# AIM-Harvard/pyradiomics

Measured on AMD Instinct MI355X. Metric: Mvoxels/s for GLCM+GLRLM build, 512^3 vol @32 bins, higher is better.
Workload: dtype u8 levels / u32 counts / f64 out; 1 GPU; GLCM+GLRLM matrix build, 512^3 int32+uint8 volume resident in HBM, 32 grey levels, full mask, 13 angles, uniform levels; one volume per GPU (batch sharding, no collective); size=512, levels=32, dist=uniform, deferred_mode=pipeline

## Files before the change

### pyradiomics_amd/csrc/kernels_sweep.h

```cpp
#pragma once
#include "prad_runtime.h"

namespace prad {

typedef unsigned int u32;
typedef unsigned long long u64;

__global__ void __launch_bounds__(256) pack_levels_kernel(const int *__restrict__ image,
                                                          const uint8_t *__restrict__ mask, long long n, int NX,
                                                          int pitch, int padw, int Ng,
                                                          uint8_t *__restrict__ levels, int *__restrict__ flags,
                                                          int vec_ok, int shift, uint8_t *__restrict__ rowzero = nullptr) {
  const long long tid = (long long)blockIdx.x * blockDim.x + threadIdx.x;
  const long long nthreads = (long long)gridDim.x * blockDim.x;
  const bool linear = (padw == 0 && pitch == NX);
  int bad = 0;
  long long done = 0;
  if (vec_ok) {
    const long long n16 = n >> 4;
    const int upr = NX >> 4;
    const int4 *im4 = reinterpret_cast<const int4 *>(image);
    const uint4 *mk4 = reinterpret_cast<const uint4 *>(mask);
    for (long long t = tid; t < n16; t += nthreads) {
      const uint4 m = mk4[t];
// ... 462 lines not shown
  Walker<DO_GLCM, DO_GLRLM, LONG, FUSED> w[LPL];
#pragma unroll
  for (int j = 0; j < LPL; j++) w[j].init(lds, h, Nr, glrlm_acc + (size_t)D.slot * Ng * Nr, lane);
  bool seen_multi = false;
  const int lane4 = lane * LPL;
  const int NM = D.NM, NU = D.NU, NX = D.NX, du = D.du, dx = D.dx;
  const long long sU = D.sU;
  WrapGeo geo;
  geo.du = du; geo.dx = dx; geo.NU = NU; geo.NX = NX;
  geo.delta = D.sM + (long long)du * D.sU + dx;
  geo.uwrapfix = -(long long)du * NU * D.sU;

  (void)nwaves;
  for (;;) {
    int grabbed = 0;
    if (lane == 0) grabbed = atomicAdd(&work[blockIdx.y], 1);
    const int chunk = __builtin_amdgcn_readfirstlane(grabbed);
    if (chunk >= D.chunks) break;
    const int u0 = chunk / D.LXc;
    const int xfirst = (chunk - u0 * D.LXc) * CW;
    bool dead[LPL];
    bool anydead_l = false;
#pragma unroll
    for (int j = 0; j < LPL; j++) {
      dead[j] = xfirst + lane4 + j >= NX;
      anydead_l = anydead_l || dead[j];
    }
    const bool anydead = __ballot(anydead_l) != 0;
    u32 livemask = 0;
#pragma unroll
    for (int j = 0; j < LPL; j++) livemask |= dead[j] ? 0u : (0xffu << (8 * j));
#pragma unroll
    for (int j = 0; j < LPL; j++) w[j].begin_line();

    WrapPos pos;
    pos.off = (long long)u0 * sU + xfirst;
    pos.u = u0;
    pos.b = xfirst;
    pos.ent_sb = -1;
    pos.ent_uw = false;
    int t0 = 0;
    for (; t0 + U <= NM; t0 += U) {
      u32 v[U];
      bool risky_l = false;
#pragma unroll
      for (int j = 0; j < LPL; j++) risky_l = risky_l || w[j].risky(U);
      const bool quiet = !pos.ent_uw && pos.ent_sb < 0 && wrap_quiet<CW>(pos, geo, U);
      if (quiet) {
        const uint8_t *pl = L + pos.off + lane4;
#pragma unroll
        for (int k = 0; k < U; k++) {
          v[k] = load_lines<LPL>(pl);
          pl += geo.delta;
        }
        if (anydead) {
#pragma unroll
          for (int k = 0; k < U; k++) v[k] &= livemask;
        }
        pos.off += (long long)U * geo.delta;
        pos.u += U * du;
        pos.b += U * dx;
        if (LONG && __ballot(risky_l) != 0) {
#pragma unroll
          for (int k = 0; k < U; k++) {
#pragma unroll
            for (int j = 0; j < LPL; j++) w[j].template step<true>((int)((v[k] >> (8 * j)) & 0xffu));
          }
        } else {
          steps_plain_group<LPL, U>(w, v);
        }
      } else {
        int sb[U];
        bool uw[U];
#pragma unroll
        for (int k = 0; k < U; k++) {
          v[k] = load_lines<LPL>(L + pos.off + lane4) & livemask;
          sb[k] = pos.ent_sb;
          uw[k] = pos.ent_uw;
          wrap_advance<CW>(pos, geo);
        }
        if (LONG && __ballot(risky_l) != 0) seen_multi |= steps_break_group<LPL, U, true>(w, v, sb, uw, lane4);
        else seen_multi |= steps_break_group<LPL, U, false>(w, v, sb, uw, lane4);
      }
    }
    for (int t = t0; t < NM; t++) {
      const u32 v = load_lines<LPL>(L + pos.off + lane4) & livemask;
#pragma unroll
      for (int j = 0; j < LPL; j++) {
        const bool brk = pos.ent_uw || (pos.ent_sb == lane4 + j);
        const int cur = (int)((v >> (8 * j)) & 0xffu);
        seen_multi |= w[j].step_brk(cur, brk);
      }
      wrap_advance<CW>(pos, geo);
    }
#pragma unroll
    for (int j = 0; j < LPL; j++) seen_multi |= w[j].end_line();
  }
  if (DO_GLRLM && !FUSED && seen_multi) multi[D.slot] = 1;
  flush_block_hist<DO_GLCM, DO_GLRLM, FUSED>(lds, h, Nr, D.slot, glcm_acc, glrlm_acc);
}

#define PRAD_ROW_PITCH 80
template <bool DO_GLCM, bool DO_GLRLM, bool LONG, bool FUSED>
__global__ void __launch_bounds__(512) sweep_rows_kernel(const uint8_t *__restrict__ L, long long nrows, int NX,
                                                         int pitch, int slot, int Ng, int Nr, int RS,
                                                         u32 *__restrict__ glcm_acc, u32 *__restrict__ glrlm_acc,
                                                         int *__restrict__ multi, int *__restrict__ flags) {
  extern __shared__ u32 lds[];
  if (flags[0]) return;
  const HistLayout h = hist_layout(DO_GLCM, DO_GLRLM, FUSED, Ng, RS);
  if (FUSED && (unsigned)(size_t)((lds_u32 *)lds) != 0u) {
    if (threadIdx.x == 0) atomicExch(flags + 2, 1);
    return;
  }
  for (int i = threadIdx.x; i < h.words; i += blockDim.x) lds[i] = 0;
  __syncthreads();
  const int lane = threadIdx.x & 63;
  const int wave = threadIdx.x >> 6;
  const int wpb = blockDim.x >> 6;
  uint8_t *tile = reinterpret_cast<uint8_t *>(lds + ((h.words + 3) & ~3)) + (size_t)wave * 64 * PRAD_ROW_PITCH;
  const long long ngroups = (nrows + 63) / 64;
  const long long nwaves = (long long)gridDim.x * wpb;
  Walker<DO_GLCM, DO_GLRLM, LONG, FUSED> w;
  w.init(lds, h, Nr, glrlm_acc + (size_t)slot * Ng * Nr, lane);
  bool seen_multi = false;
  const bool vec16 = (pitch & 15) == 0 && ((uintptr_t)L & 15) == 0;

  for (long long grp = (long long)blockIdx.x * wpb + wave; grp < ngroups; grp += nwaves) {
    const long long r0 = grp * 64;
    w.begin_line();
    for (int xc = 0; xc < NX; xc += 64) {
      if (vec16) {
#pragma unroll
        for (int j = 0; j < 4; j++) {
          const int rr = j * 16 + (lane >> 2);
          const int cx = xc + (lane & 3) * 16;
          uint4 q = make_uint4(0, 0, 0, 0);
          if (r0 + rr < nrows && cx < NX) {
            q = *reinterpret_cast<const uint4 *>(L + (r0 + rr) * pitch + cx);
            const int valid = NX - cx;
            if (valid < 16) {
              u32 *qw = reinterpret_cast<u32 *>(&q);
#pragma unroll
              for (int wd = 0; wd < 4; wd++) {
                const int keep = valid - 4 * wd;
                qw[wd] = keep >= 4 ? qw[wd] : (keep <= 0 ? 0u : (qw[wd] & ((1u << (8 * keep)) - 1u)));
              }
            }
          }
          *reinterpret_cast<uint4 *>(tile + rr * PRAD_ROW_PITCH + (lane & 3) * 16) = q;
        }
      } else {
        const bool xin = xc + lane < NX;
#pragma unroll 8
        for (int rr = 0; rr < 64; rr++) {
          uint8_t b = 0;
          if (xin && r0 + rr < nrows) b = L[(r0 + rr) * pitch + xc + lane];
          tile[rr * PRAD_ROW_PITCH + lane] = b;
        }
      }
      __builtin_amdgcn_wave_barrier();
      const uint4 *row = reinterpret_cast<const uint4 *>(tile + lane * PRAD_ROW_PITCH);
#pragma unroll
      for (int q = 0; q < 4; q++) {
        const uint4 d = row[q];
        const u32 wds[4] = {d.x, d.y, d.z, d.w};
#pragma unroll
        for (int k = 0; k < 4; k++) {
          if (LONG && __ballot(w.risky(4)) != 0) {
#pragma unroll
            for (int b = 0; b < 4; b++) w.template step<true>((int)((wds[k] >> (8 * b)) & 0xffu));
          } else {
#pragma unroll
            for (int b = 0; b < 4; b++) w.template step<false>((int)((wds[k] >> (8 * b)) & 0xffu));
          }
        }
      }
      __builtin_amdgcn_wave_barrier();
    }
    seen_multi |= w.end_line();
  }
  if (DO_GLRLM && !FUSED && seen_multi) multi[slot] = 1;
  flush_block_hist<DO_GLCM, DO_GLRLM, FUSED>(lds, h, Nr, slot, glcm_acc, glrlm_acc);
}

__global__ void __launch_bounds__(64) glcm_diag_resolve_kernel(const u32 *__restrict__ glcm_acc,
                                                               const u32 *__restrict__ glrlm_acc, int Ng, int Nr,
                                                               int Na, double *__restrict__ glcm_out,
                                                               int *__restrict__ multi) {
  const int i = blockIdx.x, a = blockIdx.y, lane = threadIdx.x;
  const u32 *row = glrlm_acc + ((size_t)a * Ng + i) * Nr;
  unsigned long long pairs = 0;
  int found = 0;
  for (int r = lane; r < Nr; r += 64) {
    const u32 v = row[r];
    pairs += (unsigned long long)r * v;
    found |= (r > 0 && v != 0);
  }
  const u32 *grow = glcm_acc + ((size_t)a * Ng + i) * Ng;
  for (int j = lane; j < Ng; j += 64) found |= (grow[j] != 0);
  for (int o = 32; o > 0; o >>= 1) pairs += __shfl_xor(pairs, o);
  if (lane == 0) glcm_out[((size_t)i * Ng + i) * Na + a] = (double)pairs;
  if (__ballot(found) != 0 && lane == 0) multi[a] = 1;
}

struct AngleSet {
  int count;
  int off[PRAD_MAX_SWEEP][3];
};
template <typename T>
__global__ void __launch_bounds__(256) multi_check_kernel(AngleSet A, const T *__restrict__ L, int Nz, int Ny,
                                                          int Nx, int pitch, int *__restrict__ multi) {
  const int a = blockIdx.y;
  if (multi[a]) return;
  const int dz = A.off[a][0], dy = A.off[a][1], dx = A.off[a][2];
  const long long n = (long long)Nz * Ny * Nx, plane = (long long)Ny * Nx;
  const long long stride = (long long)gridDim.x * blockDim.x;
  for (long long i = (long long)blockIdx.x * blockDim.x + threadIdx.x; i < n; i += stride) {
    int z = (int)(i / plane);
    const int r = (int)(i - (long long)z * plane);
    int y = r / Nx, x = r - y * Nx;
    const int pz = z - dz, py = y - dy, px = x - dx;
    if ((unsigned)pz < (unsigned)Nz && (unsigned)py < (unsigned)Ny && (unsigned)px < (unsigned)Nx) continue;
    int cnt = 0;
    while ((unsigned)z < (unsigned)Nz && (unsigned)y < (unsigned)Ny && (unsigned)x < (unsigned)Nx) {
      cnt += L[((long long)z * Ny + y) * pitch + x] != 0;
      if (cnt > 1) {
        multi[a] = 1;
        return;
      }
      z += dz; y += dy; x += dx;
    }
  }
}

__global__ void finalize_glcm_kernel(const u32 *__restrict__ acc, const u32 *__restrict__ glrlm_acc, int Ng, int Nr,
                                     int Na, int diag_from_runs, double *__restrict__ out) {
  const long long idx = (long long)blockIdx.x * blockDim.x + threadIdx.x;
  const long long total = (long long)Ng * Ng * Na;
  if (idx >= total) return;
  const int a = (int)(idx % Na);
  const long long ij = idx / Na;
  const int i = (int)(ij / Ng), j = (int)(ij - (long long)i * Ng);
  if (diag_from_runs && i == j) return;
  out[idx] = (double)acc[(size_t)a * Ng * Ng + ij];
}

__global__ void __launch_bounds__(256) finalize_glcm_diag_kernel(const u32 *__restrict__ glcm_acc, u32 *glrlm_acc, int Ng, int Nr,
                                                                 int Na, int nb1, double *__restrict__ glcm_out,
                                                                 int *__restrict__ multi, int restore_from = -1) {
  if ((int)blockIdx.x < nb1) {
    const long long idx = (long long)blockIdx.x * blockDim.x + threadIdx.x;
    const long long total = (long long)Ng * Ng * Na;
    if (idx >= total) return;
    const int a = (int)(idx % Na);
    const long long ij = idx / Na;
    const int i = (int)(ij / Ng), j = (int)(ij - (long long)i * Ng);
    if (i == j) return;
    glcm_out[idx] = (double)glcm_acc[(size_t)a * Ng * Ng + ij];
    return;
  }
  const int pair = ((int)blockIdx.x - nb1) * 4 + (int)(threadIdx.x >> 6), lane = threadIdx.x & 63;
  if (pair >= Ng * Na) return;
  const int i = pair % Ng, a = pair / Ng;
  u32 *row = glrlm_acc + ((size_t)a * Ng + i) * Nr;
  unsigned long long pairs = 0, longer = 0;
  int found = 0;
  for (int r = lane; r < Nr; r += 64) {
    const u32 v = row[r];
    pairs += (unsigned long long)r * v;
    if (r > 0) longer += v;
    found |= (r > 0 && v != 0);
  }
  const u32 *grow = glcm_acc + ((size_t)a * Ng + i) * Ng;
  for (int j = lane; j < Ng; j += 64) found |= (grow[j] != 0);
  for (int o = 32; o > 0; o >>= 1) pairs += __shfl_xor(pairs, o);
  if (lane == 0) glcm_out[((size_t)i * Ng + i) * Na + a] = (double)pairs;
  if (__ballot(found) != 0 && lane == 0) multi[a] = 1;
  if (restore_from >= 0 && a != restore_from) {
    const u32 *xrow = glrlm_acc + ((size_t)restore_from * Ng + i) * Nr;
    unsigned long long nvox = 0;
    for (int r = lane; r < Nr; r += 64) nvox += (unsigned long long)(r + 1) * xrow[r];
    for (int o = 32; o > 0; o >>= 1) {
      nvox += __shfl_xor(nvox, o);
      longer += __shfl_xor(longer, o);
    }
    if (lane == 0) row[0] = (u32)(nvox - (pairs + longer));
  }
}

__global__ void finalize_glrlm_kernel(const u32 *__restrict__ acc, const int *__restrict__ multi, int Ng, int Nr,
                                      int Na, double *__restrict__ out, const int *__restrict__ flags = nullptr,
                                      int *__restrict__ sticky = nullptr) {
  if (sticky && blockIdx.x == 0 && threadIdx.x == 0 && (flags[0] || flags[2])) sticky[0] = 1;
  const long long idx = (long long)blockIdx.x * blockDim.x + threadIdx.x;
  const long long total = (long long)Ng * Nr * Na;
  if (idx >= total) return;
  const int a = (int)(idx % Na);
  const long long gr = idx / Na;
  const int r = (int)(gr % Nr);
  out[idx] = (r == 0 && !multi[a]) ? 0.0 : (double)acc[(size_t)a * Ng * Nr + gr];
}

}
```

### pyradiomics_amd/csrc/prad_api.hip

```cpp
#include "prad_runtime.h"
#include "kernels_generic.h"
#include "kernels_pairs.h"
#include "kernels_sweep.h"
#include "kernels_sweepfw.h"
#include "kernels_sweepfw2.h"
#include "kernels_neigh.h"
#include "kernels_glszm.h"
#include "kernels_voxel.h"
#include "kernels_voxslide.h"
#include "kernels_mcc.h"
#include "kernels_voxtex.h"
#include "kernels_binning.h"

#include <algorithm>
#include <atomic>
#include <chrono>
#include <cmath>
#include <condition_variable>
#include <cstdlib>
#include <deque>
#include <limits>
#include <mutex>
#include <thread>

// ... 558 lines not shown
  return launch_lines_lpl<G, R, LNG, F, 1>(k, p, levels, Ng, Nr, glcm_acc, glrlm_acc, multi);
}

template <bool LNG, int K, bool HASPAD, bool PACK>
int launch_fw_kpp(Call &k, const SweepPlan &p, const PackJob &pj, const uint8_t *levels, const uint8_t *rowzero, int Ng, int Nr,
                  u32 *glcm_acc, u32 *glrlm_acc, int *multi, int *flags_d) {
  const size_t lds = p.fw_xblocks > 0 ? std::max(p.lds_fw, p.lds_fw_rows) : p.lds_fw;
  PRAD_HIP(hipFuncSetAttribute(reinterpret_cast<const void *>(&sweep_fw_kernel<LNG, K, HASPAD, PACK>),
                               hipFuncAttributeMaxDynamicSharedMemorySize, (int)lds));
  hipLaunchKernelGGL((sweep_fw_kernel<LNG, K, HASPAD, PACK>), dim3(p.fw_blocks + p.fw_xblocks), dim3(p.fw_threads), lds, k.s, p.fwset, pj,
                     levels, rowzero, Ng, Nr, p.RSfw, glcm_acc, glrlm_acc, multi + 2 * PRAD_MAX_SWEEP + PRAD_FW_WORK_STRIDE, flags_d);
  return check_launch("sweep_fw_kernel");
}
template <bool LNG, int K, bool HASPAD>
int launch_fw_kp(Call &k, const SweepPlan &p, const PackJob &pj, const uint8_t *levels, const uint8_t *rowzero, int Ng, int Nr,
                 u32 *glcm_acc, u32 *glrlm_acc, int *multi, int *flags_d) {
  if (pj.n16 > 0) return launch_fw_kpp<LNG, K, HASPAD, true>(k, p, pj, levels, rowzero, Ng, Nr, glcm_acc, glrlm_acc, multi, flags_d);
  return launch_fw_kpp<LNG, K, HASPAD, false>(k, p, pj, levels, rowzero, Ng, Nr, glcm_acc, glrlm_acc, multi, flags_d);
}
template <bool LNG, int K>
int launch_fw_k(Call &k, const SweepPlan &p, const PackJob &pj, const uint8_t *levels, const uint8_t *rowzero, int Ng, int Nr,
                u32 *glcm_acc, u32 *glrlm_acc, int *multi, int *flags_d) {
  if (p.Nx != 64 * K) return launch_fw_kp<LNG, K, true>(k, p, pj, levels, rowzero, Ng, Nr, glcm_acc, glrlm_acc, multi, flags_d);
  return launch_fw_kp<LNG, K, false>(k, p, pj, levels, rowzero, Ng, Nr, glcm_acc, glrlm_acc, multi, flags_d);
}
int launch_fw(Call &k, const SweepPlan &p, const PackJob &pj, const uint8_t *levels, const uint8_t *rowzero, int Ng, int Nr,
              u32 *glcm_acc, u32 *glrlm_acc, int *multi, int *flags_d) {
  if (p.fwK == 16)
    return p.LONGfw ? launch_fw_k<true, 16>(k, p, pj, levels, rowzero, Ng, Nr, glcm_acc, glrlm_acc, multi, flags_d)
                    : launch_fw_k<false, 16>(k, p, pj, levels, rowzero, Ng, Nr, glcm_acc, glrlm_acc, multi, flags_d);
  if (p.LONGfw) return p.fwK == 4 ? launch_fw_k<true, 4>(k, p, pj, levels, rowzero, Ng, Nr, glcm_acc, glrlm_acc, multi, flags_d)
                                : launch_fw_k<true, 8>(k, p, pj, levels, rowzero, Ng, Nr, glcm_acc, glrlm_acc, multi, flags_d);
  return p.fwK == 4 ? launch_fw_k<false, 4>(k, p, pj, levels, rowzero, Ng, Nr, glcm_acc, glrlm_acc, multi, flags_d)
                    : launch_fw_k<false, 8>(k, p, pj, levels, rowzero, Ng, Nr, glcm_acc, glrlm_acc, multi, flags_d);
}

template <bool LNG, int K, bool HASPAD, bool SKIP1, bool PACK>
int launch_fw2_khsp(Call &k, const SweepPlan &p, const PackJob &pj, const uint8_t *levels16, int Ng, int Nr, u32 *glcm_acc, u32 *glrlm_acc,
                    int *work, int *flags_d) {
  PRAD_HIP(hipFuncSetAttribute(reinterpret_cast<const void *>(&sweep_fw2_kernel<LNG, K, HASPAD, SKIP1, PACK>),
                               hipFuncAttributeMaxDynamicSharedMemorySize, (int)p.lds_fw2));
  hipLaunchKernelGGL((sweep_fw2_kernel<LNG, K, HASPAD, SKIP1, PACK>), dim3(p.fw_blocks), dim3(1024), p.lds_fw2, k.s, p.fwset, pj, levels16,
                     Ng, Nr, p.RS2, p.fw2_copies, glcm_acc, glrlm_acc, work, flags_d);
  return check_launch("sweep_fw2_kernel");
}
template <bool LNG, int K, bool HASPAD, bool SKIP1>
int launch_fw2_khs(Call &k, const SweepPlan &p, const PackJob &pj, const uint8_t *levels16, int Ng, int Nr, u32 *glcm_acc, u32 *glrlm_acc,
                   int *work, int *flags_d) {
  if (pj.n16 > 0) return launch_fw2_khsp<LNG, K, HASPAD, SKIP1, true>(k, p, pj, levels16, Ng, Nr, glcm_acc, glrlm_acc, work, flags_d);
  return launch_fw2_khsp<LNG, K, HASPAD, SKIP1, false>(k, p, pj, levels16, Ng, Nr, glcm_acc, glrlm_acc, work, flags_d);
}
template <bool LNG, int K>
int launch_fw2_k(Call &k, const SweepPlan &p, const PackJob &pj, const uint8_t *levels16, int Ng, int Nr, u32 *glcm_acc, u32 *glrlm_acc,
                 int *multi, int *flags_d) {
  int *work = multi + 2 * PRAD_MAX_SWEEP + PRAD_FW_WORK_STRIDE;
  if (p.Nx != 64 * K)
    return p.skip1 ? launch_fw2_khs<LNG, K, true, true>(k, p, pj, levels16, Ng, Nr, glcm_acc, glrlm_acc, work, flags_d)
                   : launch_fw2_khs<LNG, K, true, false>(k, p, pj, levels16, Ng, Nr, glcm_acc, glrlm_acc, work, flags_d);
  return p.skip1 ? launch_fw2_khs<LNG, K, false, true>(k, p, pj, levels16, Ng, Nr, glcm_acc, glrlm_acc, work, flags_d)
                 : launch_fw2_khs<LNG, K, false, false>(k, p, pj, levels16, Ng, Nr, glcm_acc, glrlm_acc, work, flags_d);
}
int launch_fw2(Call &k, const SweepPlan &p, const PackJob &pj, const uint8_t *levels16, int Ng, int Nr, u32 *glcm_acc, u32 *glrlm_acc,
               int *multi, int *flags_d) {
  if (p.LONGfw2) return p.fwK == 4 ? launch_fw2_k<true, 4>(k, p, pj, levels16, Ng, Nr, glcm_acc, glrlm_acc, multi, flags_d)
                                 : launch_fw2_k<true, 8>(k, p, pj, levels16, Ng, Nr, glcm_acc, glrlm_acc, multi, flags_d);
  return p.fwK == 4 ? launch_fw2_k<false, 4>(k, p, pj, levels16, Ng, Nr, glcm_acc, glrlm_acc, multi, flags_d)
                    : launch_fw2_k<false, 8>(k, p, pj, levels16, Ng, Nr, glcm_acc, glrlm_acc, multi, flags_d);
}

template <bool LNG>
int launch_fw_rows(Call &k, const SweepPlan &p, const uint8_t *levels, int Ng, int Nr, u32 *glcm_acc, u32 *glrlm_acc, int *flags_d) {
  const long long nrows = (long long)p.Nz * p.Ny, groups = fw_row_groups(nrows);
  const int wpb = p.fw_rows_threads / 64;
  const unsigned gx = (unsigned)std::max<long long>(1, std::min<long long>((groups + wpb - 1) / wpb, (long long)cu_count()));
  PRAD_HIP(hipFuncSetAttribute(reinterpret_cast<const void *>(&sweep_fw_rows_kernel<LNG>),
                               hipFuncAttributeMaxDynamicSharedMemorySize, (int)p.lds_fw_rows));
  hipLaunchKernelGGL((sweep_fw_rows_kernel<LNG>), dim3(gx), dim3(p.fw_rows_threads), p.lds_fw_rows, k.s, levels, nrows, p.Nx,
                     p.pitch, p.row_slot, Ng, Nr, p.RSfw_rows, glcm_acc, glrlm_acc, flags_d);
  return check_launch("sweep_fw_rows_kernel");
}

template <bool LNG>
int launch_fw2_rows(Call &k, const SweepPlan &p, const uint8_t *levels16, int Ng, int Nr, u32 *glcm_acc, u32 *glrlm_acc, int *flags_d) {
  const long long nrows = (long long)p.Nz * p.Ny, groups = nrows >= 4096 ? ((nrows + 511) / 512) * 8 : (nrows + 63) / 64;
  const int wpb = p.fw2r_waves;
  const unsigned gx = (unsigned)std::max<long long>(1, std::min<long long>((groups + wpb - 1) / wpb, (long long)cu_count()));
  PRAD_HIP(hipFuncSetAttribute(reinterpret_cast<const void *>(&sweep_fw2_rows_kernel<LNG>),
                               hipFuncAttributeMaxDynamicSharedMemorySize, (int)p.lds_fw2_rows));
  hipLaunchKernelGGL((sweep_fw2_rows_kernel<LNG>), dim3(gx), dim3(64 * wpb), p.lds_fw2_rows, k.s, levels16, nrows, p.Nx, p.pitch16,
                     p.row_slot, Ng, Nr, p.RS2r, p.fw2r_copies, glcm_acc, glrlm_acc, flags_d);
  return check_launch("sweep_fw2_rows_kernel");
}

template <bool G, bool R, bool LNG, bool F>
int launch_rows(Call &k, const SweepPlan &p, const uint8_t *levels, int Ng, int Nr, u32 *glcm_acc, u32 *glrlm_acc,
                int *multi) {
  const long long nrows = (long long)p.Nz * p.Ny;
  const long long groups = (nrows + 63) / 64;
  const int wpb = kRowsThreads / 64;
  const int per_cu = std::max(1, std::min(2048 / kRowsThreads, (int)(160 * 1024 / p.lds_bytes_rows)));
  const unsigned gx = (unsigned)std::max<long long>(1, std::min<long long>((groups + wpb - 1) / wpb, (long long)cu_count() * per_cu));
  PRAD_HIP(hipFuncSetAttribute(reinterpret_cast<const void *>(&sweep_rows_kernel<G, R, LNG, F>),
                               hipFuncAttributeMaxDynamicSharedMemorySize, (int)p.lds_bytes_rows));
  hipLaunchKernelGGL((sweep_rows_kernel<G, R, LNG, F>), dim3(gx), dim3(kRowsThreads), p.lds_bytes_rows, k.s, levels,
                     nrows, p.Nx, p.pitch, p.row_slot, Ng, Nr, p.RSr, glcm_acc, glrlm_acc, multi, k.flags_d);
  return check_launch("sweep_rows_kernel");
}

__global__ void __launch_bounds__(256) zero3_kernel(u32 *__restrict__ a, size_t na, u32 *__restrict__ b, size_t nb,
                                                    u32 *__restrict__ c3, size_t nc) {
  const size_t t = (size_t)blockIdx.x * blockDim.x + threadIdx.x, nt = (size_t)gridDim.x * blockDim.x;
  uint4 *a4 = reinterpret_cast<uint4 *>(a);
  for (size_t i = t; i < na / 4; i += nt) a4[i] = make_uint4(0, 0, 0, 0);
  for (size_t i = (na & ~(size_t)3) + t; i < na; i += nt) a[i] = 0;
  for (size_t i = t; i < nb; i += nt) b[i] = 0;
  for (size_t i = t; i < nc; i += nt) c3[i] = 0;
}

struct VolState {
  bool valid = false;
  SweepPlan p;
  int Ng = 0, Nr = 0, Na = 0;
  double *glcm = nullptr, *glrlm = nullptr;
  uint8_t *levels = nullptr, *rowzero = nullptr;
  uint8_t *levels16 = nullptr;
  u32 *acc = nullptr, *glcm_acc = nullptr, *glrlm_acc = nullptr;
  int *multi = nullptr;
  int *flags_d = nullptr;
  bool packed_inline = false;
  int lane = -1;
};

bool fin_side() {
  static const bool on = getenv("PRAD_FINALIZE_STREAM") != nullptr && atoi(getenv("PRAD_FINALIZE_STREAM")) != 0;
  return on;
}
int fin_wait_for_lane(hipStream_t s, int lane);

int vol_prepare(Call &k, const SweepPlan &p, int Ng, int Nr, double *glcm, double *glrlm, VolState &v) {
  Context &c = *k.c;
  if (fin_side() && c.lane >= 0) PRAD_TRY(fin_wait_for_lane(k.s, c.lane));
  v.lane = c.lane;
  v.valid = true;
  v.p = p;
  v.Ng = Ng;
  v.Nr = Nr;
  v.Na = k.Na;
  v.glcm = glcm;
  v.glrlm = glrlm;
  v.flags_d = k.flags_d;
  const long long nrows = (long long)p.Nz * p.Ny;
  v.levels = nullptr;
  if (!(p.fw2 && p.fw2_rows && p.lines.count > 0 && p.row_slot >= 0) || getenv("PRAD_FW2_KEEP8")) {
    PRAD_TRY(c.get<uint8_t>("levels", (size_t)nrows * p.pitch + 1024, &v.levels));
    v.levels += 512;
  }
  v.levels16 = nullptr;
  if (p.fw2) {
    PRAD_TRY(c.get<uint8_t>("levels16", (size_t)nrows * p.pitch16 + 4096, &v.levels16));
    v.levels16 += 2048;
  }
  const size_t nglcm = glcm ? (size_t)k.Na * Ng * Ng : 0, nglrlm = glrlm ? (size_t)k.Na * Ng * Nr : 0;
  const size_t nctl = 2 * PRAD_MAX_SWEEP + (size_t)PRAD_FW_WORK_STRIDE * (PRAD_FW_DOMAINS * PRAD_MAX_SWEEP + 1);
  PRAD_TRY(c.get<u32>("sweep_acc", nglcm + nglrlm + nctl, &v.acc));
  v.glcm_acc = v.acc;
  v.glrlm_acc = v.acc + nglcm;
  v.multi = (int *)(v.acc + nglcm + nglrlm);
  v.rowzero = nullptr;
  if (p.fw) PRAD_TRY(c.get<uint8_t>("rowzero", (size_t)nrows + 64, &v.rowzero));
  const size_t acc_w = nglcm + nglrlm + nctl, rz_w = v.rowzero ? ((size_t)nrows + 3) / 4 : 0;
  const size_t total_w = acc_w + rz_w + 4;
  const unsigned gx = (unsigned)std::max<size_t>(1, std::min<size_t>((total_w / 4 + 255) / 256, 1024));
  hipLaunchKernelGGL(zero3_kernel, dim3(gx), dim3(256), 0, k.s, v.acc, acc_w, reinterpret_cast<u32 *>(v.rowzero), rz_w,
                     reinterpret_cast<u32 *>(v.flags_d), (size_t)4);
  return check_launch("zero3_kernel");
}

bool pipeline_volume(const SweepPlan &p, bool glcm, bool glrlm) {
  if (!(p.ok && p.lines.count > 0 && glcm && glrlm)) return false;
  return (p.fw && p.fused) || (p.fw2 && !getenv("PRAD_FW2_LANES"));
}
bool pack_inline_ok(const Call &k, const VolState &v) {
  if (!(v.glcm && v.glrlm && v.p.pitch == v.p.Nx && v.p.padw == 0 && (k.g.n % 16) == 0 &&
        ((((uintptr_t)k.image) | ((uintptr_t)k.mask) | ((uintptr_t)v.levels)) & 15) == 0))
    return false;
  if (k.g.n >= (1LL << 31)) return false;
  if (v.p.fw2) return v.levels16 && v.p.pitch16 == 2 * v.p.Nx && (((uintptr_t)v.levels16) & 15) == 0;
  return v.p.fw && v.p.fused;
}

PackJob make_pack_job(const Call &k, const VolState &v, const VolState *host) {
  PackJob j;
  memset(&j, 0, sizeof(j));
  j.image = k.image;
  j.mask = k.mask;
  j.levels = v.levels;
  j.levels16 = v.p.fw2 ? v.levels16 : nullptr;
  j.rowzero = v.rowzero;
  j.flags = v.flags_d;
  j.n16 = k.g.n / 16;
  j.NX = v.p.Nx;
  j.Ng = v.Ng;
  double groups = 0, waves = 16.0;
  if (host) {
    for (int i = 0; i < host->p.fwset.count; i++) groups += (double)host->p.fwset.d[i].NM * host->p.fwset.d[i].NU / PRAD_FW_U;
    waves = 16.0 * std::max(1, host->p.fw_blocks);
  }
  const double units = (double)j.n16 / 64.0;
  const double slack = v.p.fw2 ? 1.05 : 0.92;
  j.every = (int)std::max(1.0, std::min(64.0, std::floor(slack * groups / std::max(1.0, units))));
  (void)waves;
  if (const char *e = getenv("PRAD_PACK_EVERY")) j.every = std::max(1, atoi(e));
  return j;
}

int vol_pack_standalone(Call &k, VolState &v) {
  Context &c = *k.c;
  const SweepPlan &p = v.p;
  Timed t(c, "pack", k.s);
  if (p.fw2) {
    const unsigned gx = (unsigned)std::max<long long>(1, std::min<long long>((k.g.n / 4 + 255) / 256, 8192));
    hipLaunchKernelGGL(pack_levels16_kernel, dim3(gx), dim3(256), 0, k.s, k.image, k.mask, k.g.n, p.Nx, p.pitch16, p.pitch, v.Ng,
                       v.levels16, v.levels, v.flags_d);
    return check_launch("pack_levels16_kernel");
  }
  const int vec_ok = p.vec_rows && ((((uintptr_t)k.image) | ((uintptr_t)k.mask) | ((uintptr_t)v.levels)) & 15) == 0;
  const unsigned gx = (unsigned)std::max<long long>(1, std::min<long long>((k.g.n / 16 + 255) / 256, 4096));
  const int shift = (v.glcm && v.glrlm && p.fused) ? PRAD_FUSED_SHIFT : 0;
  hipLaunchKernelGGL(pack_levels_kernel, dim3(gx), dim3(256), 0, k.s, k.image, k.mask, k.g.n, p.Nx, p.pitch, p.padw,
                     v.Ng, v.levels, v.flags_d, vec_ok, shift, v.rowzero);
  return check_launch("pack_levels_kernel");
}

template <bool G, bool R, bool F>
int launch_sweeps(Call &k, const VolState &v, const PackJob &pj) {
  const SweepPlan &p = v.p;
  if (p.lines.count > 0 && p.fw && G && R && F) {
    {
      Timed t(*k.c, "sweep", k.s);
      PRAD_TRY(launch_fw(k, p, pj, v.levels, v.rowzero, v.Ng, v.Nr, v.glcm_acc, v.glrlm_acc, v.multi, v.flags_d));
    }
    if (p.row_slot >= 0 && p.fw_xblocks == 0) {
      Timed t(*k.c, "rows", k.s);
      if (p.RSfw_rows < v.Nr) PRAD_TRY(launch_fw_rows<true>(k, p, v.levels, v.Ng, v.Nr, v.glcm_acc, v.glrlm_acc, v.flags_d));
      else PRAD_TRY(launch_fw_rows<false>(k, p, v.levels, v.Ng, v.Nr, v.glcm_acc, v.glrlm_acc, v.flags_d));
    }
    return PRAD_OK;
  }
  if (p.fw2 && G && R && !F && p.lines.count > 0) {
    {
      Timed t(*k.c, "sweep", k.s);
      PRAD_TRY(launch_fw2(k, p, pj, v.levels16, v.Ng, v.Nr, v.glcm_acc, v.glrlm_acc, v.multi, v.flags_d));
    }
    if (p.row_slot >= 0) {
      Timed t(*k.c, "rows", k.s);
      if (p.fw2_rows) {
        if (p.LONGfw2r) PRAD_TRY(launch_fw2_rows<true>(k, p, v.levels16, v.Ng, v.Nr, v.glcm_acc, v.glrlm_acc, v.flags_d));
        else PRAD_TRY(launch_fw2_rows<false>(k, p, v.levels16, v.Ng, v.Nr, v.glcm_acc, v.glrlm_acc, v.flags_d));
      } else if (p.LONGr) {
        PRAD_TRY((launch_rows<G, R, true, F>(k, p, v.levels, v.Ng, v.Nr, v.glcm_acc, v.glrlm_acc, v.multi)));
      } else {
        PRAD_TRY((launch_rows<G, R, false, F>(k, p, v.levels, v.Ng, v.Nr, v.glcm_acc, v.glrlm_acc, v.multi)));
      }
    }
    return PRAD_OK;
  }
  Timed t(*k.c, "sweep", k.s);
  if (p.lines.count > 0) {
    if (R && p.LONG) PRAD_TRY((launch_lines<G, R, true, F>(k, p, v.levels, v.Ng, v.Nr, v.glcm_acc, v.glrlm_acc, v.multi)));
    else PRAD_TRY((launch_lines<G, R, false, F>(k, p, v.levels, v.Ng, v.Nr, v.glcm_acc, v.glrlm_acc, v.multi)));
  }
  if (p.row_slot >= 0) {
    if (R && p.LONGr) PRAD_TRY((launch_rows<G, R, true, F>(k, p, v.levels, v.Ng, v.Nr, v.glcm_acc, v.glrlm_acc, v.multi)));
    else PRAD_TRY((launch_rows<G, R, false, F>(k, p, v.levels, v.Ng, v.Nr, v.glcm_acc, v.glrlm_acc, v.multi)));
  }
  return PRAD_OK;
}

int vol_sweep(Call &k, const VolState &v, const PackJob &pj) {
  if (pj.n16 > 0 && !pipeline_volume(v.p, v.glcm != nullptr, v.glrlm != nullptr))
    return fail(PRAD_E_ARG, "internal: a pack job needs a fixed-window host launch");
  if (pj.n16 > 0 && (pj.levels16 != nullptr) != v.p.fw2)
    return fail(PRAD_E_ARG, "internal: the pack job's layout is not the host launch's");
  if (v.glcm && v.glrlm && v.p.fused) return launch_sweeps<true, true, true>(k, v, pj);
  if (v.glcm && v.glrlm) return launch_sweeps<true, true, false>(k, v, pj);
  if (v.glcm) return launch_sweeps<true, false, false>(k, v, pj);
  return launch_sweeps<false, true, false>(k, v, pj);
}

__global__ void latch_flags_kernel(const int *__restrict__ flags, int *__restrict__ sticky) {
  if (flags[0] || flags[2]) sticky[0] = 1;
}

__global__ void latch_any_flag_kernel(const int *__restrict__ flags, int *__restrict__ sticky) {
  if (flags[0] || flags[1] || flags[2]) sticky[0] = 1;
}
int latch_neigh(Context &c, Call &k) {
  int *sticky = nullptr;
  PRAD_TRY(c.get<int>("deferred_sticky", 16, &sticky));
  hipLaunchKernelGGL(latch_any_flag_kernel, dim3(1), dim3(1), 0, k.s, (const int *)k.flags_d, sticky);
  return check_launch("latch_any_flag_kernel");
}

int vol_finalize(Call &k, const VolState &v, int *sticky) {
  Context &c = *k.c;
  const SweepPlan &p = v.p;
  const int Ng = v.Ng, Nr = v.Nr, Na = v.Na;
  double *glcm = v.glcm, *glrlm = v.glrlm;
  bool latched = false;
  {
    Timed t(c, "finalize", k.s);
    const bool runs_diag = p.fused || p.fw2;
    if (p.fw2 && p.skip1 && p.lines.count > 0 && !(glcm && glrlm && p.row_slot >= 0))
      return fail(PRAD_E_UNSUPPORTED, "sweep plan derives runs of length 1 but the call cannot restore them");
    if (glcm && glrlm && runs_diag) {
      const int nb1 = (int)blocks_for((long long)Ng * Ng * Na), nb2 = (Ng * Na + 3) / 4;
      hipLaunchKernelGGL(finalize_glcm_diag_kernel, dim3(nb1 + nb2), dim3(256), 0, k.s, v.glcm_acc, v.glrlm_acc, Ng, Nr, Na, nb1,
                         glcm, v.multi, (p.fw2 && p.skip1 && p.lines.count > 0) ? p.row_slot : -1);
      PRAD_TRY(check_launch("finalize_glcm_diag_kernel"));
    } else if (glcm) {
      hipLaunchKernelGGL(finalize_glcm_kernel, dim3(blocks_for((long long)Ng * Ng * Na)), dim3(256), 0, k.s,
                         v.glcm_acc, v.glrlm_acc, Ng, Nr, Na, p.fused ? 1 : 0, glcm);
      PRAD_TRY(check_launch("finalize_glcm_kernel"));
    }
    if (glrlm && runs_diag) {
      if (!glcm) {
        hipLaunchKernelGGL(glcm_diag_resolve_kernel, dim3(Ng, Na), dim3(64), 0, k.s, v.glcm_acc, v.glrlm_acc, Ng, Nr, Na,
                           glcm, v.multi);
        PRAD_TRY(check_launch("glcm_diag_resolve_kernel"));
      }
      if (v.levels)
        hipLaunchKernelGGL(multi_check_kernel<uint8_t>, dim3(128, Na), dim3(256), 0, k.s, p.aset, (const uint8_t *)v.levels, p.Nz, p.Ny,
                           p.Nx, p.pitch, v.multi);
      else
        hipLaunchKernelGGL(multi_check_kernel<unsigned short>, dim3(128, Na), dim3(256), 0, k.s, p.aset,
                           reinterpret_cast<const unsigned short *>(v.levels16), p.Nz, p.Ny, p.Nx, p.pitch16 / 2, v.multi);
      PRAD_TRY(check_launch("multi_check_kernel"));
    }
    if (glrlm) {
      hipLaunchKernelGGL(finalize_glrlm_kernel, dim3(blocks_for((long long)Ng * Nr * Na)), dim3(256), 0, k.s,
                         v.glrlm_acc, v.multi, Ng, Nr, Na, glrlm, (const int *)v.flags_d, sticky);
      PRAD_TRY(check_launch("finalize_glrlm_kernel"));
      latched = sticky != nullptr;
    }
  }
  if (sticky && !latched) {
    hipLaunchKernelGGL(latch_flags_kernel, dim3(1), dim3(1), 0, k.s, v.flags_d, sticky);
    PRAD_TRY(check_launch("latch_flags_kernel"));
  }
  return PRAD_OK;
}

int sweep_glcm_glrlm(Call &k, const SweepPlan &p, int Ng, int Nr, double *glcm, double *glrlm, bool *used) {
  Context &c = *k.c;
  VolState v;
  PRAD_TRY(vol_prepare(k, p, Ng, Nr, glcm, glrlm, v));
  PRAD_TRY(vol_pack_standalone(k, v));
  PackJob pj;
  memset(&pj, 0, sizeof(pj));
  PRAD_TRY(vol_sweep(k, v, pj));
  int *sticky = nullptr;
  if (c.deferred) PRAD_TRY(c.get<int>("deferred_sticky", 16, &sticky));
  PRAD_TRY(vol_finalize(k, v, sticky));
  if (c.deferred) {
    *used = true;
    return PRAD_OK;
  }
  PRAD_TRY(read_flags(k));
  *used = (k.flags_h[0] == 0 && k.flags_h[2] == 0);
  return PRAD_OK;
}

struct PipeState {
  VolState pending;
  hipStream_t s = nullptr;
  unsigned long long seq = 0;
  hipEvent_t ev = nullptr;
  int mode = -1;
  hipStream_t fin = nullptr;
  hipEvent_t fin_in = nullptr, fin_all = nullptr, fin_done[4] = {};
  bool fin_used[4] = {};
};
PipeState &pipe_state() {
  static thread_local PipeState p;
  return p;
}
bool pipeline_mode() {
  PipeState &ps = pipe_state();
  if (ps.mode < 0) {
    const char *e = getenv("PRAD_DEFERRED_MODE");
    ps.mode = (e && strcmp(e, "lanes") == 0) ? 0 : 1;
  }
  return ps.mode == 1;
}
int pipeline_sticky(Context &c, int **sticky) { return c.get<int>("deferred_sticky", 16, sticky); }

int pipeline_retire(Context &c, hipStream_t s, const PackJob &pj) {
  PipeState &ps = pipe_state();
  if (ps.s != s) {
    if (!ps.ev) PRAD_HIP(hipEventCreateWithFlags(&ps.ev, hipEventDisableTiming));
    PRAD_HIP(hipEventRecord(ps.ev, ps.s));
    PRAD_HIP(hipStreamWaitEvent(s, ps.ev, 0));
  }
  Call k;
  k.c = &c;
  k.s = s;
  k.Na = ps.pending.Na;
  k.flags_d = ps.pending.flags_d;
  int *sticky = nullptr;
  PRAD_TRY(pipeline_sticky(c, &sticky));
  PRAD_TRY(vol_sweep(k, ps.pending, pj));
  if (fin_side() && ps.pending.lane >= 0 && ps.pending.lane < 4) {
    if (!ps.fin) {
      PRAD_HIP(hipStreamCreateWithFlags(&ps.fin, hipStreamNonBlocking));
      PRAD_HIP(hipEventCreateWithFlags(&ps.fin_in, hipEventDisableTiming));
      PRAD_HIP(hipEventCreateWithFlags(&ps.fin_all, hipEventDisableTiming));
      for (int l = 0; l < 4; l++) PRAD_HIP(hipEventCreateWithFlags(&ps.fin_done[l], hipEventDisableTiming));
    }
    PRAD_HIP(hipEventRecord(ps.fin_in, s));
    PRAD_HIP(hipStreamWaitEvent(ps.fin, ps.fin_in, 0));
    Call k2 = k;
    k2.s = ps.fin;
    PRAD_TRY(vol_finalize(k2, ps.pending, sticky));
    PRAD_HIP(hipEventRecord(ps.fin_done[ps.pending.lane], ps.fin));
    ps.fin_used[ps.pending.lane] = true;
  } else {
    PRAD_TRY(vol_finalize(k, ps.pending, sticky));
  }
  ps.pending.valid = false;
  return PRAD_OK;
}

int fin_wait_for_lane(hipStream_t s, int lane) {
  PipeState &ps = pipe_state();
  if (lane < 0 || lane >= 4 || !ps.fin || !ps.fin_used[lane]) return PRAD_OK;
  PRAD_HIP(hipStreamWaitEvent(s, ps.fin_done[lane], 0));
  return PRAD_OK;
}
int fin_join(hipStream_t s, bool host) {
  PipeState &ps = pipe_state();
  if (!ps.fin) return PRAD_OK;
  if (host) {
    PRAD_HIP(hipStreamSynchronize(ps.fin));
    return PRAD_OK;
  }
  PRAD_HIP(hipEventRecord(ps.fin_all, ps.fin));
  PRAD_HIP(hipStreamWaitEvent(s, ps.fin_all, 0));
  return PRAD_OK;
}

int pipeline_flush(Context &c) {
  PipeState &ps = pipe_state();
  if (!ps.pending.valid) return PRAD_OK;
  PackJob none;
  memset(&none, 0, sizeof(none));
  const size_t before = c.times.size();
  PRAD_TRY(pipeline_retire(c, ps.s, none));
  if (c.timing_accumulate) c.all_times.insert(c.all_times.end(), c.times.begin() + (long)before, c.times.end());
  return PRAD_OK;
}

int pipeline_step(Call &k, const SweepPlan &p, int Ng, int Nr, double *glcm, double *glrlm, bool *handled) {
  Context &c = *k.c;
  PipeState &ps = pipe_state();
  *handled = false;
  if (!pipeline_volume(p, glcm != nullptr, glrlm != nullptr)) return pipeline_flush(c);
  VolState v;
  PRAD_TRY(vol_prepare(k, p, Ng, Nr, glcm, glrlm, v));
  PackJob pj;
  memset(&pj, 0, sizeof(pj));
  bool inl = false;
  if (ps.pending.valid) {
    inl = pack_inline_ok(k, v) && ps.pending.p.fw2 == v.p.fw2 && !getenv("PRAD_NO_INLINE_PACK");
    if (inl) pj = make_pack_job(k, v, &ps.pending);
    PRAD_TRY(pipeline_retire(c, k.s, pj));
  }
  if (!inl) PRAD_TRY(vol_pack_standalone(k, v));
  v.packed_inline = inl;
  ps.pending = v;
  ps.s = k.s;
  *handled = true;
  return PRAD_OK;
}

int pairs_glcm_glrlm(Call &k, int Ng, int Nr, double *glcm, double *glrlm, bool *used) {
  *used = false;
  Context &c = *k.c;
  if (k.vm.voxels || k.g.nd > 3 || Ng < 1 || Ng > PRAD_PAIR_LDS_WORDS || k.Na > PRAD_PAIR_MAXA || k.g.n >= 0x7fffffffLL ||
      getenv("PRAD_NO_PAIRS"))
    return PRAD_OK;
  int dims[3] = {1, 1, 1};
  for (int d = 0; d < k.g.nd; d++) dims[3 - k.g.nd + d] = k.g.size[d];
  PairAngles A;
  memset(&A, 0, sizeof(A));
  A.n = k.Na;
  for (int a = 0; a < k.Na; a++)
    for (int d = 0; d < k.g.nd; d++) {
      const int o = k.angles_h[a * k.g.nd + d];
      if (o < -127 || o > 127) return PRAD_OK;
      A.o[a][3 - k.g.nd + d] = (signed char)o;
    }
  if (glrlm && Nr < std::max(dims[0], std::max(dims[1], dims[2]))) return PRAD_OK;
  const size_t gwords = glcm ? (size_t)k.Na * Ng * Ng : 0, rwords = glrlm ? (size_t)k.Na * Ng * Nr : 0;
  if ((gwords + rwords) * sizeof(u32) > ((size_t)1 << 30)) return PRAD_OK;
  hipStream_t s = k.s;
  lev16 *L = nullptr;
  u32 *gacc = nullptr, *racc = nullptr, *counts = nullptr;
  int *multi = nullptr;
  PRAD_TRY(c.get<lev16>("pairs_levels", (size_t)k.g.n + 8, &L));
  if (glcm) PRAD_TRY(c.get<u32>("pairs_glcm_acc", gwords, &gacc));
  if (glrlm) {
    PRAD_TRY(c.get<u32>("pairs_glrlm_acc", rwords, &racc));
    PRAD_TRY(c.get<u32>("pairs_counts", (size_t)Ng, &counts));
    PRAD_TRY(c.get<int>("pairs_multi", (size_t)PRAD_PAIR_MAXA, &multi));
  }
  PRAD_HIP(hipMemsetAsync(k.flags_d, 0, sizeof(int) * 4, s));
  const int cus = cu_count();
  {
    Timed t(c, "pack", s);
    const unsigned gx = (unsigned)std::max<long long>(1, std::min<long long>((k.g.n + 255) / 256, (long long)cus * 16));
    hipLaunchKernelGGL(pairs_pack_kernel, dim3(gx), dim3(256), 0, s, k.image, k.mask, k.g.n, Ng, L, k.flags_d);
    PRAD_TRY(check_launch("pairs_pack_kernel"));
  }
  if (glcm) {
    Timed t(c, "pairs", s);
    PRAD_HIP(hipMemsetAsync(gacc, 0, sizeof(u32) * gwords, s));
    int AG, RT, ntile;
    if ((long long)Ng * Ng <= PRAD_PAIR_LDS_WORDS) {
      AG = std::max(1, std::min(k.Na, PRAD_PAIR_LDS_WORDS / (Ng * Ng)));
      RT = Ng;
      ntile = 1;
    } else {
      AG = 1;
      RT = PRAD_PAIR_LDS_WORDS / Ng;
      ntile = (Ng + RT - 1) / RT;
    }
    const int npass = ((k.Na + AG - 1) / AG) * ntile;
    const size_t lds = sizeof(u32) * (size_t)AG * RT * Ng;
    PRAD_HIP(hipFuncSetAttribute(reinterpret_cast<const void *>(&pairs_glcm_kernel), hipFuncAttributeMaxDynamicSharedMemorySize, (int)lds));
    long long gbest = 1;
    double ebest = 0;
    for (long long gtry = std::max<long long>(1, 2LL * cus / npass); gtry <= std::max<long long>(1, (4LL * cus + npass - 1) / npass); gtry++) {
      const long long total = gtry * npass, rounds = (total + cus - 1) / cus;
      const double eff = (double)total / (double)(rounds * cus);
      if (eff > ebest + 1e-9) {
        ebest = eff;
        gbest = gtry;
      }
    }
    const unsigned gx = (unsigned)std::max<long long>(1, std::min<long long>((k.g.n / 8 + 1023) / 1024, gbest));
    hipLaunchKernelGGL(pairs_glcm_kernel, dim3(gx, (unsigned)npass), dim3(1024), lds, s, L, dims[0], dims[1], dims[2], A, AG, RT,
                       ntile, Ng, gacc, k.flags_d);
    PRAD_TRY(check_launch("pairs_glcm_kernel"));
    const long long total = (long long)Ng * Ng * k.Na;
    hipLaunchKernelGGL(finalize_glcm_kernel, dim3(blocks_for(total)), dim3(256), 0, s, gacc, (const u32 *)nullptr, Ng, 1, k.Na, 0, glcm);
    PRAD_TRY(check_launch("finalize_glcm_kernel"));
  }
  if (glrlm) {
    Timed t(c, "pairs", s);
    PRAD_HIP(hipMemsetAsync(racc, 0, sizeof(u32) * rwords, s));
    PRAD_HIP(hipMemsetAsync(counts, 0, sizeof(u32) * (size_t)Ng, s));
    PRAD_HIP(hipMemsetAsync(multi, 0, sizeof(int) * PRAD_PAIR_MAXA, s));
    const int use_lds = Ng <= 8192;
    const unsigned gc = (unsigned)std::max<long long>(1, std::min<long long>((k.g.n + 255) / 256, (long long)cus * 8));
    hipLaunchKernelGGL(pairs_level_count_kernel, dim3(gc), dim3(256), use_lds ? sizeof(u32) * (size_t)Ng : 0, s, L, k.g.n, Ng, use_lds,
                       counts, k.flags_d);
    PRAD_TRY(check_launch("pairs_level_count_kernel"));
    const unsigned gx = (unsigned)std::max<long long>(1, std::min<long long>((k.g.n + 255) / 256, std::max(1LL, 16LL * cus / k.Na)));
    hipLaunchKernelGGL(pairs_glrlm_kernel, dim3(gx, (unsigned)k.Na), dim3(256), 0, s, L, dims[0], dims[1], dims[2], A, Ng, Nr, racc, multi,
                       k.flags_d);
    PRAD_TRY(check_launch("pairs_glrlm_kernel"));
    hipLaunchKernelGGL(pairs_multi_check_kernel, dim3(gx, (unsigned)k.Na), dim3(256), 0, s, A, L, dims[0], dims[1], dims[2], multi, k.flags_d);
    PRAD_TRY(check_launch("pairs_multi_check_kernel"));
    hipLaunchKernelGGL(pairs_run1_kernel, dim3((unsigned)((Ng * k.Na + 3) / 4)), dim3(256), 0, s, racc, counts, Ng, Nr, k.Na, k.flags_d);
    PRAD_TRY(check_launch("pairs_run1_kernel"));
    const long long total = (long long)Ng * Nr * k.Na;
    hipLaunchKernelGGL(finalize_glrlm_kernel, dim3(blocks_for(total)), dim3(256), 0, s, racc, multi, Ng, Nr, k.Na, glrlm,
                       (const int *)nullptr, (int *)nullptr);
    PRAD_TRY(check_launch("finalize_glrlm_kernel"));
  }
  PRAD_TRY(read_flags(k));
  *used = k.flags_h[0] == 0;
  if (!*used) {
    PRAD_HIP(hipMemsetAsync(k.flags_d, 0, sizeof(int) * 4, s));
  }
  return PRAD_OK;
}

int texture_pairs_runs(const int32_t *image, const uint8_t *mask, const int *size, int Nd, const int *angles,
                       int Na, int Ng, int Nr, int Nvox, const int *voxels, int kernelRadius, int force2Ddim,
                       double *glcm, double *glrlm, hipStream_t s) {
  if (!glcm && !glrlm) return fail(PRAD_E_ARG, "both outputs are NULL");
  if (Ng < 1 || (glrlm && Nr < 1)) return fail(PRAD_E_ARG, "Ng/Nr must be >= 1");
  Context &c = ctx();
  PRAD_TRY(c.ensure_device());
  struct LaneGuard {
    Context &c;
    ~LaneGuard() { c.lane = -1; }
  } lane_guard{c};
  bool pipe = c.deferred && !voxels && pipeline_mode();
  if (c.deferred && !voxels && !pipe) PRAD_TRY(c.lane_begin(s, &s));
  if (pipe) c.lane = (int)(pipe_state().seq++ % (fin_side() ? 3u : 2u));
  Call k;
  PRAD_TRY(setup_call(k, image, mask, size, Nd, angles, Na, Nvox, voxels, kernelRadius, force2Ddim, s, false));
  SweepPlan p = plan_sweep(k, Ng, Nr, glcm != nullptr, glrlm != nullptr);
  if (pipe && !pipeline_volume(p, glcm != nullptr, glrlm != nullptr)) {
    const hipStream_t user = s;
    PRAD_TRY(pipeline_flush(c));
    pipe = false;
    c.lane = -1;
    PRAD_TRY(c.lane_begin(user, &s));
    if (c.lane >= 0) c.lane += fin_side() ? 3 : 2;
    PRAD_TRY(setup_call(k, image, mask, size, Nd, angles, Na, Nvox, voxels, kernelRadius, force2Ddim, s, false));
    p = plan_sweep(k, Ng, Nr, glcm != nullptr, glrlm != nullptr);
  }
  PRAD_TRY(c.begin_call(s));
  if (!p.ok) PRAD_HIP(hipMemsetAsync(k.flags_d, 0, sizeof(int) * 4, s));
// ... 1340 lines not shown
```

Measured before the change: 291,700 Mvoxels/s.

## Fuse GLCM/GLRLM finalize, diagonal resolve and multi-check into one kernel

Adds a single finalize_volume_kernel that, in one launch, copies off-diagonal GLCM entries, copies GLRLM entries for runs longer than one, resolves the GLCM diagonal and run-length-1 counts per angle, and performs the multi-voxel line check only when the accumulators show no evidence of it. This replaces several separate finalize, resolve and multi-check launches, cutting launch overhead and the unconditional full-volume scan in the multi check. The cost is more complex per-angle block logic with shared-memory atomics. The fused path is on by default and can be turned off with an environment variable.

```diff
diff --git a/pyradiomics_amd/csrc/kernels_sweep.h b/pyradiomics_amd/csrc/kernels_sweep.h
--- a/pyradiomics_amd/csrc/kernels_sweep.h
+++ b/pyradiomics_amd/csrc/kernels_sweep.h
@@ -788,4 +788,151 @@
   out[idx] = (r == 0 && !multi[a]) ? 0.0 : (double)acc[(size_t)a * Ng * Nr + gr];
 }
 
-}
+
+template <typename T>
+__device__ void lines_hold_two(const T *__restrict__ L, int Nz, int Ny, int Nx, int pitch, int dz, int dy, int dx,
+                               volatile int *hit) {
+  const int z0 = dz > 0 ? 0 : Nz - 1, y0 = dy > 0 ? 0 : Ny - 1, x0 = dx > 0 ? 0 : Nx - 1;
+  const long long NzR = Nz - (dz != 0), NyR = Ny - (dy != 0);
+  const long long SZ = dz ? (long long)Ny * Nx : 0, SY = dy ? NzR * Nx : 0, SX = dx ? NzR * NyR : 0;
+  const long long dp = ((long long)dz * Ny + dy) * pitch + dx;
+  for (long long s = threadIdx.x; s < SZ + SY + SX; s += blockDim.x) {
+    if (*hit) return;
+    int z, y, x;
+    if (s < SZ) {
+      z = z0;
+      y = (int)(s / Nx);
+      x = (int)(s - (long long)y * Nx);
+    } else if (s < SZ + SY) {
+      const long long t = s - SZ;
+      const int zr = (int)(t / Nx);
+      x = (int)(t - (long long)zr * Nx);
+      y = y0;
+      z = zr + (dz > 0);
+    } else {
+      const long long t = s - SZ - SY;
+      const int zr = (int)(t / NyR);
+      x = x0;
+      y = (int)(t - zr * NyR) + (dy > 0);
+      z = zr + (dz > 0);
+    }
+    int len = 0x7fffffff;
+    if (dz) len = min(len, dz > 0 ? Nz - z : z + 1);
+    if (dy) len = min(len, dy > 0 ? Ny - y : y + 1);
+    if (dx) len = min(len, dx > 0 ? Nx - x : x + 1);
+    long long p = ((long long)z * Ny + y) * pitch + x;
+    int cnt = 0;
+    for (int k = 0; k < len; k += 8, p += 8 * dp) {
+#pragma unroll
+      for (int u = 0; u < 8; u++)
+        if (k + u < len) cnt += L[p + u * dp] != 0;
+      if (cnt > 1) {
+        *hit = 1;
+        return;
+      }
+    }
+  }
+}
+
+template <typename T>
+__global__ void __launch_bounds__(1024) finalize_volume_kernel(AngleSet A, const T *__restrict__ L, int Nz, int Ny, int Nx, int pitch,
+                                                               const u32 *__restrict__ glcm_acc, u32 *glrlm_acc,
+                                                               int Ng, int Nr, int Na, int nbR, double *__restrict__ glcm_out,
+                                                               double *__restrict__ glrlm_out, int *__restrict__ multi,
+                                                               int restore_from, const int *__restrict__ flags,
+                                                               int *__restrict__ sticky) {
+  __shared__ u64 s_pairs[256], s_longer[256], s_nvox[256];
+  __shared__ u32 s_run1[256];
+  __shared__ int s_found, s_hit;
+  const int b = blockIdx.x, tid = threadIdx.x;
+  if (b >= Na + nbR) {
+    const long long idx = (long long)(b - Na - nbR) * blockDim.x + tid;
+    if (idx >= (long long)Ng * Ng * Na) return;
+    const int a = (int)(idx % Na);
+    const long long ij = idx / Na;
+    const int i = (int)(ij / Ng), j = (int)(ij - (long long)i * Ng);
+    if (i == j) return;
+    glcm_out[idx] = (double)glcm_acc[(size_t)a * Ng * Ng + ij];
+    return;
+  }
+  if (b >= Na) {
+    const long long idx = (long long)(b - Na) * blockDim.x + tid;
+    if (idx >= (long long)Ng * Nr * Na) return;
+    const int a = (int)(idx % Na);
+    const long long gr = idx / Na;
+    if (gr % Nr == 0) return;
+    glrlm_out[idx] = (double)glrlm_acc[(size_t)a * Ng * Nr + gr];
+    return;
+  }
+  const int a = b, lane = tid & 63, nt = (int)blockDim.x;
+  const int nrun = Ng * Nr, npair = Ng * Ng;
+  const bool restore = restore_from >= 0 && a != restore_from;
+  const u32 *gtab = glcm_acc + (size_t)a * npair;
+  u32 g[8];
+#pragma unroll
+  for (int u = 0; u < 8; u++) g[u] = (u * nt + tid < npair) ? gtab[u * nt + tid] : 0u;
+  for (int i = tid; i < 256; i += nt) {
+    s_pairs[i] = 0;
+    s_longer[i] = 0;
+    s_nvox[i] = 0;
+    s_run1[i] = 0;
+  }
+  if (tid == 0) {
+    s_found = multi[a] != 0;
+    s_hit = 0;
+    if (sticky && a == 0 && (flags[0] || flags[2])) sticky[0] = 1;
+  }
+  __syncthreads();
+  int found = 0;
+  u32 *tab = glrlm_acc + (size_t)a * nrun;
+  const u32 *xtab = glrlm_acc + (size_t)(restore ? restore_from : a) * nrun;
+  for (int e0 = 0; e0 < nrun; e0 += 16 * nt) {
+    u32 v[16], x[16];
+#pragma unroll
+    for (int u = 0; u < 16; u++) v[u] = (e0 + u * nt + tid < nrun) ? tab[e0 + u * nt + tid] : 0u;
+#pragma unroll
+    for (int u = 0; u < 16; u++) x[u] = (restore && e0 + u * nt + tid < nrun) ? xtab[e0 + u * nt + tid] : 0u;
+#pragma unroll
+    for (int u = 0; u < 16; u++)
+      if (v[u] | x[u]) {
+        const int e = e0 + u * nt + tid, i = e / Nr, r = e - i * Nr;
+        if (x[u]) atomicAdd(&s_nvox[i], (u64)(r + 1) * x[u]);
+        if (v[u] && r == 0) {
+          s_run1[i] = v[u];
+        } else if (v[u]) {
+          found = 1;
+          atomicAdd(&s_pairs[i], (u64)r * v[u]);
+          atomicAdd(&s_longer[i], (u64)v[u]);
+        }
+      }
+  }
+#pragma unroll
+  for (int u = 0; u < 8; u++) found |= (g[u] != 0);
+  for (int e0 = 8 * nt; e0 < npair; e0 += 8 * nt) {
+#pragma unroll
+    for (int u = 0; u < 8; u++) g[u] = (e0 + u * nt + tid < npair) ? gtab[e0 + u * nt + tid] : 0u;
+#pragma unroll
+    for (int u = 0; u < 8; u++) found |= (g[u] != 0);
+  }
+  if (__ballot(found) != 0 && lane == 0) s_found = 1;
+  __syncthreads();
+  int m = s_found;
+  if (!m) {
+    lines_hold_two<T>(L, Nz, Ny, Nx, pitch, A.off[a][0], A.off[a][1], A.off[a][2], &s_hit);
+    __syncthreads();
+    m = s_hit;
+  }
+  for (int i = tid; i < Ng; i += nt) {
+    const u64 pairs = s_pairs[i];
+    glcm_out[((size_t)i * Ng + i) * Na + a] = (double)pairs;
+    u32 run1 = s_run1[i];
+    if (restore) {
+      run1 = (u32)(s_nvox[i] - (pairs + s_longer[i]));
+      tab[(size_t)i * Nr] = run1;
+    }
+    glrlm_out[(size_t)i * Nr * Na + a] = m ? (double)run1 : 0.0;
+  }
+  if (tid == 0) multi[a] = m;
+}
+
+}
diff --git a/pyradiomics_amd/csrc/prad_api.hip b/pyradiomics_amd/csrc/prad_api.hip
--- a/pyradiomics_amd/csrc/prad_api.hip
+++ b/pyradiomics_amd/csrc/prad_api.hip
@@ -884,6 +884,11 @@
   return check_launch("latch_any_flag_kernel");
 }
 
+bool finalize_one() {
+  const char *e = getenv("PRAD_FINALIZE_ONE");
+  return !(e && atoi(e) == 0 && e[0] != '\0');
+}
+
 int vol_finalize(Call &k, const VolState &v, int *sticky) {
   Context &c = *k.c;
   const SweepPlan &p = v.p;
@@ -895,6 +900,21 @@
     const bool runs_diag = p.fused || p.fw2;
     if (p.fw2 && p.skip1 && p.lines.count > 0 && !(glcm && glrlm && p.row_slot >= 0))
       return fail(PRAD_E_UNSUPPORTED, "sweep plan derives runs of length 1 but the call cannot restore them");
+    if (glcm && glrlm && runs_diag && finalize_one() && (long long)Ng * Nr < (1LL << 30)) {
+      const int nbR = (int)blocks_for((long long)Ng * Nr * Na, 1024), nbG = (int)blocks_for((long long)Ng * Ng * Na, 1024);
+      const int restore_from = (p.fw2 && p.skip1 && p.lines.count > 0) ? p.row_slot : -1;
+      if (v.levels)
+        hipLaunchKernelGGL(finalize_volume_kernel<uint8_t>, dim3(Na + nbR + nbG), dim3(1024), 0, k.s, p.aset, (const uint8_t *)v.levels,
+                           p.Nz, p.Ny, p.Nx, p.pitch, v.glcm_acc, v.glrlm_acc, Ng, Nr, Na, nbR, glcm, glrlm, v.multi,
+                           restore_from, (const int *)v.flags_d, sticky);
+      else
+        hipLaunchKernelGGL(finalize_volume_kernel<unsigned short>, dim3(Na + nbR + nbG), dim3(1024), 0, k.s, p.aset,
+                           reinterpret_cast<const unsigned short *>(v.levels16), p.Nz, p.Ny, p.Nx, p.pitch16 / 2, v.glcm_acc,
+                           v.glrlm_acc, Ng, Nr, Na, nbR, glcm, glrlm, v.multi, restore_from, (const int *)v.flags_d, sticky);
+      PRAD_TRY(check_launch("finalize_volume_kernel"));
+      latched = sticky != nullptr;
+      glcm = glrlm = nullptr;
+    }
     if (glcm && glrlm && runs_diag) {
       const int nb1 = (int)blocks_for((long long)Ng * Ng * Na), nb2 = (Ng * Na + 3) / 4;
       hipLaunchKernelGGL(finalize_glcm_diag_kernel, dim3(nb1 + nb2), dim3(256), 0, k.s, v.glcm_acc, v.glrlm_acc, Ng, Nr, Na, nb1,
```

Result: faster. 294,700 Mvoxels/s, median of 6 (+1.0%).
